# mbway/turbo

Hardware: AMD Instinct MI355X
Metric: acquisition evals/sec (M candidates, N training) + GP-fit ms (higher is better)
Workload: dtype f32

## Files before the change

turbo_amd/csrc/prune_screen_h2.hpp:

```cpp
#pragma once
#include <hip/hip_runtime.h>
#include <math.h>

#include "prune_screen.hpp"
#include "trmm_f16x2.hpp"

namespace tgp {

constexpr int SCRH_MIN_D = 15;
constexpr int SCRH_ROW = 144;
constexpr int SCRH_MAXEXP = 40;

struct ScreenH2Terms { double dcoef, P, Qc, Qw; };
inline ScreenH2Terms screen_h2_error_terms(double constant, int D, int N) {
    const double u = 0x1p-24, ce = 1.001 * constant, L = fabs(log2(constant));
    ScreenH2Terms t;
    t.dcoef = 2.01 * D + 25.0 + 0.26 * sqrt((double)D);
    t.P = ce * u * 0.5 * t.dcoef;
    t.Qc = screen_error_terms(constant, D, N).Q + ce * (0.7 * L * u + 0x1p-41);
    t.Qw = t.Qc + ce * u * (2.4 + 1.4 * L);
    return t;
}

__host__ __device__ inline double screen_h2_weight(double dcoef, double R) {
    const double delta = dcoef * 0x1p-24 * R + 0x1p-40;
    return delta <= 1.0 ? 1.001 * expm1(0.5001 * delta) : INFINITY;
}
__host__ __device__ inline double screen_h2_error(double closed, double wcoef, double W, double wadd) {
    return fmin(closed, wcoef * W + wadd);
}

__host__ __device__ inline float screen_h2_scale(float m) {
    int e;
    frexpf(m, &e);
    int ex = 14 - e;
    ex = ex > SCRH_MAXEXP ? SCRH_MAXEXP : (ex < -SCRH_MAXEXP ? -SCRH_MAXEXP : ex);
    return ldexpf(1.f, ex);
}

struct ScreenH2Scal {
    double ea, eb, wadd;
    float nxmax, sx;
    int npos, nneg, ok, pad;
};

struct ScreenH2PrepArgs {
    const float *Xs;
    const double *alpha;
    int N, Dp, nch;
    long ncap;
    double P, Qc, Qw;
    unsigned char *Xh;
    float *nxp, *absa;
    ScreenH2Scal *scal;
};

__global__ __launch_bounds__(256) void screen_h2_prep_kernel(ScreenH2PrepArgs a) {
    __shared__ double sa[256];
    __shared__ float smx[256], smn[256];
    __shared__ int spos[256], sbef[256], sbad[256];
    __shared__ int wcnt[4];
    const int tid = threadIdx.x, base = blockIdx.x * 256;
    const int N = a.N, Dp = a.Dp;
    double a1 = 0.0;
    float mxx = 0.f, mxn = 0.f;
    int npos = 0, before = 0, bad = 0;
    for (int i = tid; i < N; i += 256) {
        const float *row = a.Xs + (long)i * Dp;
        double s = 0.0;
        float m = 0.f;
        for (int d = 0; d < Dp; d += 4) {
            const f4_t x = *reinterpret_cast<const f4_t *>(row + d);
#pragma unroll
            for (int e = 0; e < 4; ++e) { s = fma((double)x[e], (double)x[e], s); m = fmaxf(m, fabsf(x[e])); }
        }
        if (!(s < (double)INFINITY)) bad = 1;
        mxn = fmaxf(mxn, (float)s);
        mxx = fmaxf(mxx, m);
        const double al = a.alpha[i];
        a1 += fabs(al);
        const int p = al >= 0.0;
        npos += p;
        if (i < base) before += p;
    }
    sa[tid] = a1; smx[tid] = mxx; smn[tid] = mxn; spos[tid] = npos; sbef[tid] = before; sbad[tid] = bad;
    __syncthreads();
    for (int o = 128; o > 0; o >>= 1) {
        if (tid < o) {
            sa[tid] += sa[tid + o];
            smx[tid] = fmaxf(smx[tid], smx[tid + o]);
            smn[tid] = fmaxf(smn[tid], smn[tid + o]);
            spos[tid] += spos[tid + o];
            sbef[tid] += sbef[tid + o];
            sbad[tid] |= sbad[tid + o];
        }
        __syncthreads();
    }
    npos = spos[0];
    before = sbef[0];
    const int nneg = N - npos, np128 = (npos + 127) & ~127, nn128 = (nneg + 127) & ~127;
    const float xm2 = 2.f * smx[0];
    const float sx = xm2 > 0.f ? screen_h2_scale(xm2) : 1.f;
    const int ok = !sbad[0] && xm2 < 0x1p54f;
    if (blockIdx.x == 0 && tid == 0) {
        const double an = 1.001 * sa[0];
        ScreenH2Scal s;
        s.ea = an * (a.P * (double)smn[0] + a.Qc);
        s.eb = an * a.P;
        s.wadd = an * a.Qw;
        s.nxmax = smn[0]; s.sx = sx;
        s.npos = npos; s.nneg = nneg; s.ok = ok; s.pad = 0;
        *a.scal = s;
    }

    const int i = base + tid;
    const bool live = i < N;
    const double al = live ? a.alpha[i] : -1.0;
    const bool pos = live && al >= 0.0;
    const unsigned long long bal = __ballot(pos);
    const int lane = tid & 63, w = tid >> 6;
    if (lane == 0) wcnt[w] = __popcll(bal);
    __syncthreads();
    int pre = __popcll(bal & ((1ull << lane) - 1ull));
    for (int k = 0; k < w; ++k) pre += wcnt[k];
    auto write_row = [&](long dest, const float *row, float absal) {
        double s = 0.0;
        for (int ch = 0; ch < a.nch; ++ch) {
            unsigned h[2][16];
#pragma unroll
            for (int q = 0; q < 8; ++q) {
                const int d = ch * SCR_DC + 4 * q;
                f4_t x = {0.f, 0.f, 0.f, 0.f};
                if (row && d < Dp) x = *reinterpret_cast<const f4_t *>(row + d);
#pragma unroll
                for (int e = 0; e < 4; ++e) s = fma((double)x[e], (double)x[e], s);
                split2_f16x2(-2.f * x[0], -2.f * x[1], sx, h[0][2 * q], h[1][2 * q]);
                split2_f16x2(-2.f * x[2], -2.f * x[3], sx, h[0][2 * q + 1], h[1][2 * q + 1]);
            }
            unsigned char *o = a.Xh + ((long)ch * a.ncap + dest) * 128;
#pragma unroll
            for (int pl = 0; pl < 2; ++pl)
#pragma unroll
                for (int q = 0; q < 4; ++q)
                    *reinterpret_cast<u4_t *>(o + 64 * pl + 16 * q) = (u4_t){h[pl][4 * q], h[pl][4 * q + 1], h[pl][4 * q + 2], h[pl][4 * q + 3]};
        }
        a.nxp[dest] = (float)s;
        a.absa[dest] = absal;
    };
    if (live) write_row(pos ? before + pre : np128 + (i - before - pre), a.Xs + (long)i * Dp, (float)fabs(al));
    if (blockIdx.x == 0 && tid < 128) {
        if (npos + tid < np128) write_row(npos + tid, nullptr, 0.f);
        if (nneg + tid < nn128) write_row(np128 + nneg + tid, nullptr, 0.f);
    }
}

struct ScreenH2Args {
    const float *Cs;
    const unsigned char *Xh;
    const float *nxp, *absa;
    const ScreenH2Scal *scal;
    double *mupart, *wpart;
    double *err, *wcoef;
    long ldpart, ncap;
    int Dp;
    double constant, dcoef;
};

__global__ __launch_bounds__(256, 2) void prune_screen_h2_kernel(ScreenH2Args g) {
    __shared__ __attribute__((aligned(16))) unsigned char Ct[SCR_T * SCRH_ROW];
    __shared__ __attribute__((aligned(16))) unsigned char Xt[SCR_T * SCRH_ROW];
    __shared__ __attribute__((aligned(16))) f4_t rowc[SCR_T];
    __shared__ float srow[SCR_T];
    __shared__ double mpos[SCR_T];
    const int tid = threadIdx.x, lane = tid & 63, w = tid >> 6;
    const int li = lane & 31, lh = lane >> 5;
    const long c0 = (long)blockIdx.x * SCR_T;
    const int Dp = g.Dp;
    const ScreenH2Scal sc = *g.scal;
    const int ntp = (sc.npos + SCR_T - 1) / SCR_T;
    const int njt = ntp + (sc.nneg + SCR_T - 1) / SCR_T;
    const int per = (njt + (int)gridDim.y - 1) / (int)gridDim.y;
    const int jt0 = blockIdx.y * per;
    const int jt1 = jt0 + per < njt ? jt0 + per : njt;
    const int nch = (Dp + SCR_DC - 1) / SCR_DC;
    const int nsteps = (jt1 > jt0 ? jt1 - jt0 : 0) * nch;
    const bool one_pass = nch == 1;
    constexpr float KAPPA = -0.72134752044448170368f;

    if (tid < SCR_T) {
        const float *row = g.Cs + (c0 + tid) * Dp;
        double s = 0.0;
        float m = 0.f;
        for (int d = 0; d < Dp; d += 4) {
            const f4_t x = *reinterpret_cast<const f4_t *>(row + d);
#pragma unroll
            for (int e = 0; e < 4; ++e) { s = fma((double)x[e], (double)x[e], s); m = fmaxf(m, fabsf(x[e])); }
        }
        const double R = s + (double)sc.nxmax;
        const bool ok = sc.ok && R < 0x1p46;
        const float sr = ok ? (m > 0.f ? screen_h2_scale(m) : 1.f) : 0.f;
        const float S = sr * sc.sx;
        srow[tid] = sr;
        rowc[tid] = (f4_t){S, KAPPA / S, (float)((double)log2f((float)g.constant) + (double)KAPPA * s), -(float)((double)S * s)};
        if (blockIdx.y == 0) {
            g.err[c0 + tid] = ok ? sc.ea + sc.eb * s : (double)INFINITY;
            g.wcoef[c0 + tid] = ok ? screen_h2_weight(g.dcoef, R) : (double)INFINITY;
        }
    }
    __syncthreads();
    ScrStage sp;
    u4_t xq[4];
    auto store_c = [&]() {
#pragma unroll
        for (int p = 0; p < 4; ++p) {
            const int idx = tid + 256 * p;
            const int r = idx >> 3, dv = (idx & 7) * 4;
            const float sr = srow[r];
            unsigned a0, a1, b0, b1;
            split2_f16x2(sp.v[p][0], sp.v[p][1], sr, a0, b0);
            split2_f16x2(sp.v[p][2], sp.v[p][3], sr, a1, b1);
            *reinterpret_cast<uint2 *>(Ct + r * SCRH_ROW + 2 * dv) = make_uint2(a0, a1);
            *reinterpret_cast<uint2 *>(Ct + r * SCRH_ROW + 64 + 2 * dv) = make_uint2(b0, b1);
        }
    };
    auto load_x = [&](int jt, int ch) {
        const unsigned char *src = g.Xh + ((long)ch * g.ncap + (long)jt * SCR_T) * 128;
#pragma unroll
        for (int p = 0; p < 4; ++p) xq[p] = *reinterpret_cast<const u4_t *>(src + (tid + 256 * p) * 16);
    };
    auto store_x = [&]() {
#pragma unroll
        for (int p = 0; p < 4; ++p) {
            const int idx = tid + 256 * p;
            *reinterpret_cast<u4_t *>(Xt + (idx >> 3) * SCRH_ROW + (idx & 7) * 16) = xq[p];
        }
    };
    if (nsteps > 0) {
        sp.load(g.Cs, c0, Dp, 0);
        load_x(jt0, 0);
        store_c();
        store_x();
    }
    __syncthreads();
    double sum[16];
#pragma unroll
    for (int r = 0; r < 16; ++r) sum[r] = 0.0;
    auto mma = [](u4_t a, u4_t b, f16_t c) {
        return __builtin_amdgcn_mfma_f32_32x32x16_f16(__builtin_bit_cast(f16x8_t, a), __builtin_bit_cast(f16x8_t, b), c, 0, 0, 0);
    };
    f16_t hi[4], mid[4];
    for (int st = 0; st < nsteps; ++st) {
        const int jt = jt0 + st / nch, ch = st - (st / nch) * nch;
        const int j0 = jt * SCR_T;
        const bool more = st + 1 < nsteps;
        if (more) {
            const int jn = jt0 + (st + 1) / nch, cn = (st + 1) - ((st + 1) / nch) * nch;
            load_x(jn, cn);
        }
        float nxv[4], al[4];
        if (ch == nch - 1) {
#pragma unroll
            for (int b = 0; b < 4; ++b) {
                nxv[b] = g.nxp[j0 + 32 * b + li];
                al[b] = g.absa[j0 + 32 * b + li];
            }
        }
        if (ch == 0) {
            if (jt == ntp && jt > jt0) {
#pragma unroll
                for (int r = 0; r < 16; ++r) {
                    double s = sum[r];
#pragma unroll
                    for (int o = 16; o > 0; o >>= 1) s += __shfl_xor(s, o, 64);
                    if (li == 0) mpos[32 * w + Mfma<float>::c_row(lane, r)] = s;
                    sum[r] = 0.0;
                }
            }
#pragma unroll
            for (int b = 0; b < 4; ++b)
#pragma unroll
                for (int r = 0; r < 16; ++r) { hi[b][r] = 0.f; mid[b][r] = 0.f; }
        }
        int dn = Dp - ch * SCR_DC;
        if (dn > SCR_DC) dn = SCR_DC;
        const int nkb = (dn + 15) >> 4;
#pragma unroll 1
        for (int kb = 0; kb < nkb; ++kb) {
            const int off = 32 * kb + 16 * lh;
            const unsigned char *ap = Ct + (32 * w + li) * SCRH_ROW + off;
            const u4_t a1 = *reinterpret_cast<const u4_t *>(ap), a2 = *reinterpret_cast<const u4_t *>(ap + 64);
#pragma unroll
            for (int b = 0; b < 4; ++b) {
                const unsigned char *bp = Xt + (32 * b + li) * SCRH_ROW + off;
                const u4_t b1 = *reinterpret_cast<const u4_t *>(bp), b2 = *reinterpret_cast<const u4_t *>(bp + 64);
                hi[b] = mma(a1, b1, hi[b]);
                mid[b] = mma(a1, b2, mid[b]);
                mid[b] = mma(a2, b1, mid[b]);
            }
        }
        if (ch == nch - 1) {
#pragma unroll
            for (int r = 0; r < 16; ++r) {
                const f4_t rc = rowc[32 * w + Mfma<float>::c_row(lane, r)];
                float p = 0.f;
#pragma unroll
                for (int b = 0; b < 4; ++b) {
                    const float t = fmaf(mid[b][r], 0x1p-11f, hi[b][r]);
                    const float s = fmaxf(fmaf(nxv[b], rc[0], t), rc[3]);
                    const float kv = __builtin_amdgcn_exp2f(fmaf(s, rc[1], rc[2]));
                    p = b == 0 ? kv * al[0] : fmaf(kv, al[b], p);
                }
                sum[r] += (double)p;
            }
        }
        if (more) {
            __syncthreads();
            if (!one_pass) {
                sp.load(g.Cs, c0, Dp, ((st + 1) - ((st + 1) / nch) * nch) * SCR_DC);
                store_c();
            }
            store_x();
            __syncthreads();
        }
    }
    const bool has_pos = nsteps > 0 && jt0 < ntp, has_neg = nsteps > 0 && jt1 > ntp;
#pragma unroll
    for (int r = 0; r < 16; ++r) {
        double s = sum[r];
#pragma unroll
        for (int o = 16; o > 0; o >>= 1) s += __shfl_xor(s, o, 64);
        if (li == 0) {
            const int row = 32 * w + Mfma<float>::c_row(lane, r);
            const double mp = has_neg ? (has_pos ? mpos[row] : 0.0) : s, mn = has_neg ? s : 0.0;
            const long o = (long)blockIdx.y * g.ldpart + c0 + row;
            g.mupart[o] = mp - mn;
            g.wpart[o] = mp + mn;
        }
    }
}

}
```

turbo_amd/csrc/sweep_pruned.hpp:

```cpp
#pragma once

namespace tgp {

struct BoundArgs {
    const double *mupart, *abspart; long ldpart; int njs;
    long m;
    double err_scale;
    const double *err;
    const double *wcoef;
    const double *wadd;
    double y_mean, y_std;
    double sig_lo, sig_hi;
    int acq; double sf, incumbent, param, margin;
    double *ub;
};

__global__ __launch_bounds__(256) void prune_bound_kernel(BoundArgs b) {
    const long c = (long)blockIdx.x * 256 + threadIdx.x;
    if (c >= b.m) return;
    double mun = 0.0, s = 0.0;
    for (int j = 0; j < b.njs; ++j) {
        mun += b.mupart[(long)j * b.ldpart + c];
        if (!b.err || b.wcoef) s += b.abspart[(long)j * b.ldpart + c];
    }
    double e = b.err ? b.err[c] : b.err_scale * s;
    if (b.wcoef) e = screen_h2_error(e, b.wcoef[c], s, b.wadd[0]);
    const double mu = b.y_std * (b.sf > 0.0 ? mun + e : mun - e) + b.y_mean;
    const double a_lo = acq_value(b.acq, b.sf, b.incumbent, b.param, mu, b.sig_lo);
    const double a_hi = acq_value(b.acq, b.sf, b.incumbent, b.param, mu, b.sig_hi);
    double a = a_lo > a_hi ? a_lo : a_hi;
    double scale = fabs(a);
    if (b.acq == TGP_ACQ_UCB) scale += fabs(mu) + fabs(b.param) * b.sig_hi;
    a += b.margin * scale;
    b.ub[c] = (isnan(a_lo) || isnan(a_hi) || isnan(a)) ? INFINITY : a;
}

__global__ __launch_bounds__(256) void prune_pick_kernel(const double *__restrict__ ub, long m, long gs,
                                                         long long *__restrict__ pick) {
    __shared__ double sv[256];
    __shared__ long long si[256];
    const long g0 = (long)blockIdx.x * gs;
    const long g1 = g0 + gs < m ? g0 + gs : m;
    Best b;
    for (long c = g0 + threadIdx.x; c < g1; c += 256) {
        const double u = ub[c];
        if (u > b.v) { b.v = u; b.i = c; }
    }
    b = block_argmax<256>(b, sv, si);
    if (threadIdx.x == 0) pick[blockIdx.x] = b.i == IDX_NONE ? g0 : b.i;
}

template <typename T>
__global__ __launch_bounds__(256) void prune_gather_kernel(const T *__restrict__ Cs, int Dp, const long long *__restrict__ idx,
                                                           long n, long rows, T *__restrict__ out) {
    const long total = rows * Dp;
    for (long i = (long)blockIdx.x * 256 + threadIdx.x; i < total; i += (long)gridDim.x * 256) {
        const long r = i / Dp;
        const int d = (int)(i - r * Dp);
        out[i] = r < n ? Cs[idx[r] * Dp + d] : (T)0;
    }
}

struct SurvArgs {
    const double *ub; long m;
    const long long *pick; long gs;
    const double *lb; double margin;
    int *bcnt; const int *boff;
    long long *sidx;
    const long long *src;
};

__device__ __forceinline__ bool prune_survives(const SurvArgs &s, long c) {
    const double lb = s.lb[0];
    const double bar = isinf(lb) ? lb : lb - s.margin * fabs(lb);
    return c < s.m && s.ub[c] >= bar && (s.src || s.pick[c / s.gs] != c);
}

__global__ __launch_bounds__(256) void prune_count_kernel(SurvArgs s) {
    __shared__ int wsum[4];
    const long c = (long)blockIdx.x * 256 + threadIdx.x;
    const unsigned long long bal = __ballot(prune_survives(s, c));
    if ((threadIdx.x & 63) == 0) wsum[threadIdx.x >> 6] = __popcll(bal);
    __syncthreads();
    if (threadIdx.x == 0) s.bcnt[blockIdx.x] = wsum[0] + wsum[1] + wsum[2] + wsum[3];
}

__global__ __launch_bounds__(1024) void prune_scan_kernel(const int *__restrict__ bcnt, int nb, int *__restrict__ boff,
                                                          long long *__restrict__ total) {
    __shared__ int part[1024];
    const int per = (nb + 1023) / 1024;
    const int b0 = (int)threadIdx.x * per;
    const int b1 = b0 + per < nb ? b0 + per : nb;
    int s = 0;
    for (int b = b0; b < b1; ++b) s += bcnt[b];
    part[threadIdx.x] = s;
    __syncthreads();
    for (int o = 1; o < 1024; o <<= 1) {
        const int v = (int)threadIdx.x >= o ? part[threadIdx.x - o] : 0;
        __syncthreads();
        part[threadIdx.x] += v;
        __syncthreads();
    }
    int run = part[threadIdx.x] - s;
    for (int b = b0; b < b1; ++b) { boff[b] = run; run += bcnt[b]; }
    if (threadIdx.x == 1023) total[0] = part[1023];
}

__global__ __launch_bounds__(256) void prune_scatter_kernel(SurvArgs s) {
    __shared__ int wsum[4];
    const long c = (long)blockIdx.x * 256 + threadIdx.x;
    const bool keep = prune_survives(s, c);
    const unsigned long long bal = __ballot(keep);
    const int lane = threadIdx.x & 63, w = threadIdx.x >> 6;
    if (lane == 0) wsum[w] = __popcll(bal);
    __syncthreads();
    int off = s.boff[blockIdx.x];
    for (int k = 0; k < w; ++k) off += wsum[k];
    if (keep) s.sidx[off + __popcll(bal & ((1ull << lane) - 1ull))] = s.src ? s.src[c] : c;
}

struct PruneWs {
    double *ub; long long *pick, *sidx, *misc; int *bcnt, *boff; void *cs;
    double *err, *ub1; long long *sidx1; float *nx;
    double *wcoef; unsigned char *xh; float *nxp, *absa; long ncap;
};
static size_t al256(size_t b) { return (b + 255) & ~(size_t)255; }

struct Carver {
    char *base = nullptr;
    size_t off = 0;
    template <typename U>
    U *take(size_t count, bool wanted = true) {
        U *ptr = base ? reinterpret_cast<U *>(base + off) : nullptr;
        if (wanted) off += al256(count * sizeof(U));
        return ptr;
    }
};

template <typename T>
static void prune_carve(const Context &c, int64_t npick, int64_t rows_cap, bool screen, bool h2, Carver &k, PruneWs &w) {
    const size_t M = (size_t)c.M, nb = (size_t)((c.M + 255) / 256), Mpad = (size_t)c.ws_Mpad;
    w.ncap = (long)((c.N + SCR_T - 1) / SCR_T + 1) * SCR_T;
    const size_t ncap = (size_t)w.ncap, nch = (size_t)((c.Dp + SCR_DC - 1) / SCR_DC);
    w.ub = k.take<double>(M);
    w.pick = k.take<long long>((size_t)npick);
    w.sidx = k.take<long long>(M);
    w.misc = k.take<long long>(32);
    w.bcnt = k.take<int>(nb);
    w.boff = k.take<int>(nb);
    w.cs = k.take<T>((size_t)rows_cap * c.Dp);
    w.err = k.take<double>(Mpad, screen);
    w.ub1 = k.take<double>((size_t)rows_cap, screen);
    w.sidx1 = k.take<long long>(M, screen);
    w.nx = k.take<float>((size_t)c.Np, screen);
    w.wcoef = k.take<double>(Mpad, h2);
    w.xh = k.take<unsigned char>(nch * ncap * 128, h2);
    w.nxp = k.take<float>(ncap, h2);
    w.absa = k.take<float>(ncap, h2);
}

template <typename T>
static hipError_t prune_workspace(Context &c, int64_t npick, int64_t rows_cap, bool screen, bool h2, PruneWs &w) {
    Carver count;
    prune_carve<T>(c, npick, rows_cap, screen, h2, count, w);
    TGP_TRY(c.d_prune.reserve(count.off, [&] { return hipStreamSynchronize(c.stream); }));
    Carver k{c.d_prune};
    prune_carve<T>(c, npick, rows_cap, screen, h2, k, w);
    return hipSuccess;
}

template <typename T>
static TrmmVariant contract_variant(const SweepPlan<T> &p, int64_t rows, int ntm) {
    TrmmVariant v;
    v.kern = p.early.kern; v.lds = trmm_glds_lds_bytes(); v.tile_m = 128; v.tile_n = 128; v.threads = 256;
    if ((rows / 128) * ntm >= CONTRACT_MIN_WGS) return v;
    if ((rows / 64) * ntm >= CONTRACT_MIN_WGS) {
        v.kern = trmm_sumsq_glds_narrow_kernel<T, 64>; v.lds = trmm_narrow_lds_bytes<64>(); v.tile_n = 64;
    } else {
        v.kern = trmm_sumsq_glds_narrow_kernel<T, 32>; v.lds = trmm_narrow_lds_bytes<32>(); v.tile_n = 32;
    }
    return v;
}

template <typename T>
static hipError_t contract_rows(Context &c, const SweepPlan<T> &p, const T *cs, int64_t n, ProfCursor &cur) {
    for (int64_t off = 0; off < n; off += c.launch_rows) {
        const int64_t m = n - off < c.launch_rows ? n - off : c.launch_rows;
        const int64_t rows = pad128(m);
        TGP_TRY(launch_kstar<T>(c, Kstar::SlabNoMean, cs + off * c.Dp, rows, p.njs, c.d_Ks[0].get(), c.d_mupart + off,
                                (long)c.Np / 16, 1.f, cur.st));
        cur.seg(1);
        TGP_TRY(launch_trmm<T>(c, p, contract_variant<T>(p, rows, p.n128), 0, off, rows, 0, p.n128, 0, true, cur.st));
        cur.seg(0, (double)m * (double)c.N * (double)c.N);
    }
    return hipSuccess;
}

enum class PruneGo { NotEligible, GatedOff, Go };
template <typename T>
static PruneGo prune_eligible(const Context &c, const SweepPlan<T> &p, const SweepCall &call) {
    const int acq = call.acq;
    if (call.mu || call.sigma || call.acqv) return PruneGo::NotEligible;
    if (acq != TGP_ACQ_EI && acq != TGP_ACQ_PI && acq != TGP_ACQ_UCB) return PruneGo::NotEligible;
    if (c.dtype != TGP_F32 && c.dtype != TGP_F64) return PruneGo::NotEligible;
    if (!p.mean_in_trmm || tuning_sweep_prune_now() == 0) return PruneGo::NotEligible;
    if (!(c.M > tuning().prune_top)) return PruneGo::NotEligible;
    if (!((double)c.M * (double)c.N * (double)c.N >= tuning_prune_min_work_now())) return PruneGo::NotEligible;
    const double u = sizeof(T) == 4 ? 0x1p-24 : 0x1p-53;
    const bool gate = c.noise > 0.0 && c.noise / (c.constant + c.noise) >= tuning().prune_tau * u;
    return gate ? PruneGo::Go : PruneGo::GatedOff;
}

template <typename T>
struct PruneRun {
    Context &c;
    const SweepPlan<T> &p;
    const SweepCall &call;
    PruneWs w;
    BoundArgs b;
    const T *Cs, *Xs;
    T *cs;
    int64_t gs, npick, keep;
    bool screen, h2;
    ProfCursor cur;
};

template <typename T>
static hipError_t tight_bound(PruneRun<T> &r, const T *rowsrc, int64_t rows, int64_t m, double *ub) {
    Context &c = r.c;
    const int njs_b = grid_splits(rows / (16 * kstar_ar(sizeof(T))), BOUND_MIN_WGS, r.p.njs, r.p.njs);
    TGP_TRY(launch_kstar<T>(c, Kstar::Bound, rowsrc, rows, njs_b, c.d_part.get(), c.d_mupart, 0L, 1.f, c.stream));
    r.cur.seg(1);
    r.b.njs = njs_b; r.b.m = m; r.b.err = nullptr; r.b.wcoef = nullptr; r.b.ub = ub;
    hipLaunchKernelGGL(prune_bound_kernel, dim3((unsigned)((m + 255) / 256)), dim3(256), 0, c.stream, r.b);
    return hipGetLastError();
}

static hipError_t screen_h2_bound(PruneRun<float> &r, int64_t xb, int njs_s) {
    Context &c = r.c;
    const PruneWs &w = r.w;
    const int N = (int)c.N, Dp = (int)c.Dp;
    const ScreenH2Terms et = screen_h2_error_terms(c.constant, (int)c.D, N);
    ScreenH2Scal *scal = reinterpret_cast<ScreenH2Scal *>(w.misc + 8);
    static_assert(sizeof(ScreenH2Scal) <= 256 - 64, "the scalars live behind misc's first eight words");
    ScreenH2PrepArgs a{};
    a.Xs = r.Xs; a.alpha = c.d_alpha; a.N = N; a.Dp = Dp; a.nch = (Dp + SCR_DC - 1) / SCR_DC; a.ncap = w.ncap;
    a.P = et.P; a.Qc = et.Qc; a.Qw = et.Qw;
    a.Xh = w.xh; a.nxp = w.nxp; a.absa = w.absa; a.scal = scal;
    hipLaunchKernelGGL(screen_h2_prep_kernel, dim3((unsigned)((N + 255) / 256)), dim3(256), 0, c.stream, a);
    TGP_TRY(hipGetLastError());
    r.cur.restart();
    ScreenH2Args g{};
    g.Cs = r.Cs; g.Xh = w.xh; g.nxp = w.nxp; g.absa = w.absa; g.scal = scal;
    g.mupart = c.d_mupart; g.wpart = c.d_part; g.err = w.err; g.wcoef = w.wcoef; g.ldpart = c.ws_Mpad; g.ncap = w.ncap;
    g.Dp = Dp; g.constant = c.constant; g.dcoef = et.dcoef;
    hipLaunchKernelGGL(prune_screen_h2_kernel, dim3((unsigned)xb, (unsigned)njs_s), dim3(256), 0, c.stream, g);
    TGP_TRY(hipGetLastError());
    r.cur.seg(2);
    c.prune_arith = 2;
    r.b.wcoef = w.wcoef; r.b.wadd = &scal->wadd;
    return hipSuccess;
}

static hipError_t screen_f32_bound(PruneRun<float> &r, int64_t xb, int njs_s) {
    Context &c = r.c;
    const PruneWs &w = r.w;
    const int N = (int)c.N, Dp = (int)c.Dp;
    const ScreenTerms et = screen_error_terms(c.constant, (int)c.D, N);
    double *scal = reinterpret_cast<double *>(w.misc + 8);
    hipLaunchKernelGGL(screen_stats_kernel, dim3(1), dim3(1024), 0, c.stream, r.Xs, c.d_alpha, N, (int)c.Np, Dp, et.P, et.Q, w.nx, scal);
    TGP_TRY(hipGetLastError());
    r.cur.restart();
    ScreenArgs g{};
    g.Cs = r.Cs; g.Xs = r.Xs; g.alpha = c.d_alpha; g.nx = w.nx; g.scal = scal;
    g.mupart = c.d_mupart; g.err = w.err; g.ldpart = c.ws_Mpad;
    g.N = N; g.Np = (int)c.Np; g.Dp = Dp; g.constant = c.constant;
    hipLaunchKernelGGL(prune_screen_kernel, dim3((unsigned)xb, (unsigned)njs_s), dim3(256), 0, c.stream, g);
    TGP_TRY(hipGetLastError());
    r.cur.seg(2);
    c.prune_arith = 1;
    r.b.wcoef = nullptr;
    return hipSuccess;
}

template <typename T>
static hipError_t bound_all(PruneRun<T> &r) {
    Context &c = r.c;
    if (!r.screen) return tight_bound<T>(r, r.Cs, c.ws_Mpad, c.M, r.w.ub);
    if constexpr (sizeof(T) == 4) {
        const int64_t xb = c.ws_Mpad / SCR_T;
        const int njt = ((int)c.N + SCR_T - 1) / SCR_T;
        const int njs_s = grid_splits(xb, SCREEN_MIN_WGS, r.p.njs, njt < r.p.njs ? njt : r.p.njs);
        TGP_TRY(r.h2 ? screen_h2_bound(r, xb, njs_s) : screen_f32_bound(r, xb, njs_s));
        r.b.njs = njs_s; r.b.m = c.M; r.b.err = r.w.err; r.b.ub = r.w.ub;
        hipLaunchKernelGGL(prune_bound_kernel, dim3((unsigned)((c.M + 255) / 256)), dim3(256), 0, c.stream, r.b);
        return hipGetLastError();
    }
    return hipSuccess;
}

template <typename T>
static hipError_t gather_rows(PruneRun<T> &r, const long long *idx, int64_t n) {
    const int Dp = (int)r.c.Dp;
    const long total = (long)pad128(n) * Dp;
    const long blocks = (total + 255) / 256 < 8192 ? (total + 255) / 256 : 8192;
    hipLaunchKernelGGL(prune_gather_kernel<T>, dim3((unsigned)blocks), dim3(256), 0, r.c.stream, r.Cs, Dp, idx, (long)n,
                       (long)pad128(n), r.cs);
    return hipGetLastError();
}

template <typename T>
static hipError_t finalize_rows(PruneRun<T> &r, const long long *idx, int64_t n, int64_t blk0) {
    FinArgs f = fin_args<T>(r.c, r.p, r.call);
    f.base_pairs = r.p.nunits;
    f.njs = 1;
    f.off = blk0 * FIN_BLOCK; f.m = n;
    f.gidx = idx;
    hipLaunchKernelGGL(finalize_kernel, dim3((unsigned)((n + FIN_BLOCK - 1) / FIN_BLOCK)), dim3(FIN_BLOCK), 0, r.c.stream, f);
    return hipGetLastError();
}

template <typename T>
static hipError_t lb_set(PruneRun<T> &r, int64_t &nblk) {
    Context &c = r.c;
    hipLaunchKernelGGL(prune_pick_kernel, dim3((unsigned)r.npick), dim3(256), 0, c.stream, r.w.ub, (long)c.M, (long)r.gs, r.w.pick);
    TGP_TRY(hipGetLastError());
    TGP_TRY(gather_rows(r, r.w.pick, r.npick));
    TGP_TRY(contract_rows<T>(c, r.p, r.cs, r.npick, r.cur));
    TGP_TRY(finalize_rows(r, r.w.pick, r.npick, 0));
    nblk = (r.npick + FIN_BLOCK - 1) / FIN_BLOCK;
    return launch_argmax(c, c.stream, (long)nblk, nullptr, nullptr, Bell{nullptr, 0, nullptr});
}

template <typename T>
static hipError_t survivors(PruneRun<T> &r, const double *ub, int64_t m, const long long *src, long long *out, long long &n) {
    Context &c = r.c;
    const PruneWs &w = r.w;
    hipStream_t st = c.stream;
    const int64_t nb = (m + 255) / 256;
    SurvArgs s{ub, (long)m, w.pick, (long)r.gs, c.d_best, r.b.margin, w.bcnt, w.boff, out, src};
    hipLaunchKernelGGL(prune_count_kernel, dim3((unsigned)nb), dim3(256), 0, st, s);
    TGP_TRY(hipGetLastError());
    hipLaunchKernelGGL(prune_scan_kernel, dim3(1), dim3(1024), 0, st, w.bcnt, (int)nb, w.boff, w.misc);
    TGP_TRY(hipGetLastError());
    hipLaunchKernelGGL(prune_scatter_kernel, dim3((unsigned)nb), dim3(256), 0, st, s);
    TGP_TRY(hipGetLastError());
    TGP_TRY(hipMemcpyAsync(&n, w.misc, sizeof(long long), hipMemcpyDeviceToHost, st));
    return hipStreamSynchronize(st);
}

template <typename T>
static hipError_t narrow_after_screen(PruneRun<T> &r, long long &nsurv, const long long *&sidx) {
    Context &c = r.c;
    const PruneWs &w = r.w;
    if (nsurv > r.keep) {
        r.cur.restart();
        TGP_TRY(tight_bound<T>(r, r.Cs, c.ws_Mpad, c.M, w.ub));
        TGP_TRY(survivors(r, w.ub, c.M, nullptr, w.sidx, nsurv));
    } else if (nsurv > tuning_prune_direct_now()) {
        TGP_TRY(gather_rows(r, w.sidx, nsurv));
        r.cur.restart();
        TGP_TRY(tight_bound<T>(r, r.cs, pad128(nsurv), nsurv, w.ub1));
        const long long n0 = nsurv;
        TGP_TRY(survivors(r, w.ub1, n0, w.sidx, w.sidx1, nsurv));
        sidx = w.sidx1;
    }
    r.cur.restart();
    return hipSuccess;
}

template <typename T>
static hipError_t contract_survivors_and_pick(PruneRun<T> &r, const long long *sidx, int64_t nsurv, int64_t nblk_lb) {
    int64_t nblk = 0;
    if (nsurv > 0) {
        TGP_TRY(gather_rows(r, sidx, nsurv));
        TGP_TRY(contract_rows<T>(r.c, r.p, r.cs, nsurv, r.cur));
        TGP_TRY(finalize_rows(r, sidx, nsurv, nblk_lb));
        nblk = (nsurv + FIN_BLOCK - 1) / FIN_BLOCK;
    }
    return launch_argmax(r.c, r.c.stream, (long)(nblk_lb + nblk), r.call.winner, r.call.res, Bell{nullptr, 0, nullptr});
}

static BoundArgs bound_args(const Context &c, const SweepCall &call, double margin) {
    BoundArgs b{};
    b.mupart = c.d_mupart; b.abspart = c.d_part; b.ldpart = c.ws_Mpad;
    b.err_scale = 4.0 * (double)((int)c.N + 8) * 0x1p-53;
    b.y_mean = c.y_mean; b.y_std = c.y_std;
    b.sig_lo = sqrt((0.99 * c.noise) * (c.y_std * c.y_std));
    b.sig_hi = sqrt((c.constant + c.noise) * (c.y_std * c.y_std));
    b.acq = call.acq; b.sf = call.sf; b.incumbent = call.incumbent; b.param = call.param; b.margin = margin;
    return b;
}

template <typename T>
static hipError_t sweep_pruned(Context &c, const SweepPlan<T> &p, const SweepCall &call, bool front_usable, bool &done) {
    done = false;
    const Tuning &tu = tuning();
    const int64_t M = c.M;
    const int64_t top = tu.prune_top < 1 ? 1 : tu.prune_top;
    const int64_t gs = (M + top - 1) / top, npick = (M + gs - 1) / gs;
    const double frac = tuning_prune_frac_now();
    const int64_t keep = frac < 0.0 ? -1 : (frac >= 1.0 ? M : (int64_t)(frac * (double)M));
    const int64_t rows_cap = pad128(npick > keep ? npick : keep);
    const bool screen = sizeof(T) == 4 && c.kernel == TGP_RBF && c.D <= SCR_MAXD && tuning_prune_screen_now() != 0;
    const bool h2 = screen && tuning_screen_arith_now() == 2 && c.D >= SCRH_MIN_D;
    PruneRun<T> r{c, p, call, PruneWs{}, BoundArgs{}, reinterpret_cast<const T *>(c.d_Cs.get()), train_points<T>(c), nullptr,
                  gs, npick, keep, screen, h2, ProfCursor{c, c.stream, -1}};
    TGP_TRY(prune_workspace<T>(c, npick, rows_cap, screen, h2, r.w));
    TGP_TRY(lds_opt_in(c, p.early.kern, p.early.lds));
    r.cs = reinterpret_cast<T *>(r.w.cs);
    c.prune_screen = -1;
    c.prune_arith = 0;
    if (!front_usable) TGP_TRY(issue_prep<T>(c, c.stream));
    r.cur.restart();
    r.b = bound_args(c, call, tu.prune_margin);

    TGP_TRY(bound_all(r));
    int64_t nblk_lb = 0;
    TGP_TRY(lb_set(r, nblk_lb));
    long long nsurv = 0;
    const long long *sidx = r.w.sidx;
    TGP_TRY(survivors(r, r.w.ub, M, nullptr, r.w.sidx, nsurv));
    c.prune_lbset = npick;
    if (screen) {
        c.prune_screen = nsurv;
        TGP_TRY(narrow_after_screen(r, nsurv, sidx));
    }
    c.prune_surv = nsurv;
    if (nsurv > keep) {
        c.prune_state = 1;
        return hipMemsetAsync(c.d_besti + 1, 0, sizeof(long long), c.stream);
    }
    TGP_TRY(contract_survivors_and_pick(r, sidx, nsurv, nblk_lb));
    c.prune_state = 0;
    done = true;
    return hipSuccess;
}

}
```

turbo_amd/csrc/tgp_internal.hpp:

```cpp
#pragma once
#include <hip/hip_runtime.h>
#include <stdint.h>

#include <string>
#include <vector>

#include "../../include/turbogp.h"
#include "dev_mem.hpp"
#include "doorbell.hpp"
#include "lds_opt_in.hpp"
#include "mes_math.hpp"
#include "tuning.hpp"

namespace tgp {


constexpr int NB = 64;
constexpr int NPAD = 256;
constexpr int SW_BM = 128;
constexpr int SW_BN = 128;
constexpr int KS_JS = 8;
constexpr int FIN_BLOCK = 256;
constexpr int CONTRACT_MIN_WGS = 512;
constexpr int SCREEN_MIN_WGS = 1024;
constexpr int BOUND_MIN_WGS = 2048;

struct ProfSeg { int a, b, kind; double flops; };

struct PreSweep {
    int mode = 0;
    int issue = 0;
    bool front = false;
    int rows128 = 0;
    long gen = -1;
    const double *cand = nullptr;
    int64_t M = 0, Mpad = 0, launch_rows = 0, chunk = 0;
    bool pending = false;
    Ev ev;
    Ev ev_in;
};

struct FitMem {
    Dev<double> d_t1, d_t2;
    Dev<double> d_Xs;
    Dev<double> d_ls;
    Dev<double> d_K;
    Dev<double> d_Linv;
    Dev<double> d_W;
    Dev<double> d_U;
    Dev<double> d_Dinv;
    Dev<double> d_Apan;
    Dev<double> d_yn;
    Dev<double> d_z;
    Dev<double> d_alpha;
    Dev<double> d_apart;
    Dev<float> d_Xs32;
    Dev<float> d_Linv32;
    Dev<unsigned short> d_Linv16;
    long linv16_gen = -1;
    Dev<unsigned> d_x2scal;
    int64_t cap_Np = 0, cap_D = 0;
    bool cap_full = false;
    int64_t linv_ld = 0;
    Dev<double> d_gpart;
    Dev<double> d_gout;
    int64_t g_cap_Np = 0, g_cap_Dp = 0;
    Dev<double> d_qws;
    Dev<double> d_rf;
    Dev<unsigned long long> d_stamp;
};

struct WsMem {
    Dev<void> d_Cs;
    Dev<void> d_Ks[2];
    Dev<double> d_part;
    Dev<double> d_mupart;
    int64_t ws_Mpad = 0;
    Dev<char> d_prune;
    Dev<double> d_topv;
    Dev<long long> d_topi;
    Dev<double> d_batch;
    Dev<double> d_bt;
    Dev<double> d_btm;
    Dev<long long> d_bti;
    Dev<double> d_ts;
    Dev<double> d_tsm;
    int64_t ts_S = 0, ts_F = 0;
    long ts_gen = -1;
    Dev<double> d_cov;
    Dev<double> d_mes;
    int mes_S = 0;
    long mes_gen = -1;
    Dev<double> d_int_a, d_int_mu, d_int_m2;
};

struct OutMem {
    Dev<double> d_mu, d_sigma, d_acq;
    int64_t out_cap = 0;
};

struct Context : FitMem, WsMem, OutMem {
    int device = 0;
    int dtype = TGP_F64;
    hipStream_t stream = nullptr;
    hipStream_t stream_own = nullptr;
    hipStream_t bg_lease = nullptr;
    hipStream_t stream_bg = nullptr;
    hipStream_t stream_pre = nullptr;
    PreSweep pre;
    std::vector<Ev> ev_la;
    Ev ev0, ev1;
    Ev evg[4];
    double last_grad_ms[3] = {0.0, 0.0, 0.0};
    std::string err;

    bool fitted = false;
    int64_t N = 0, D = 0, Np = 0;
    int64_t Dp = 0;
    int kernel = TGP_RBF;
    double constant = 1.0, noise = 0.0, jitter = 0.0;
    double y_mean = 0.0, y_std = 1.0, lml = 0.0;
    std::vector<double> ls;
    std::vector<double> h_X;
    std::vector<double> h_y;
    int normalize_y = 1;
    double sumlog = 0.0;
    Dev<double> d_scal;
    Dev<int> d_flag;
    bool grad_staged = false;
    bool grad_timed = true;
    double last_cov_ms = 0.0;
    long fit_gen = 0;
    float linv16_sb = 0.f;
    bool imported = false;
    int64_t import_rows = 0;
    int64_t fit_gen_src = -1;

    bool small = false;
    int64_t linv_extent = 0;
    Pin<double> h_pin_in{hipHostMallocMapped | hipHostMallocCoherent};
    Pin<double> h_pin_out{hipHostMallocMapped | hipHostMallocCoherent};
    Pin<double> h_pin_cand{hipHostMallocMapped};
    Pin<uint32_t> h_mt_words{hipHostMallocDefault, false};
    Ev ev_mt[2];
    Pin<unsigned long long> h_bell{hipHostMallocMapped | hipHostMallocCoherent};
    unsigned long long bell_seq = 0;
    Dev<unsigned> d_ticket;
    Dev<double> d_sfg;

    const double *d_cand = nullptr;
    Dev<double> d_cand_owned;
    int64_t M = 0;

    int64_t chunk = 0;
    int64_t launch_rows = 0;
    int prune_state = -1;
    int64_t prune_lbset = 0, prune_surv = 0;
    int64_t prune_screen = -1;
    int prune_arith = 0;
    double screen_ms = 0.0;
    Dev<double> d_bval;
    Dev<long long> d_bidx;
    double *d_winner = nullptr;
    int64_t winner_offset = 0;
    Ev ev_winner;
    bool winner_recorded = false;
    Dev<double> d_best;
    Dev<long long> d_besti;

    bool profiling = false;
    std::vector<Ev> ev_pool;
    size_t ev_used = 0;
    std::vector<ProfSeg> segs;
    int64_t trmm_launches = 0, kstar_launches = 0;
    double trmm_ms = 0.0, kstar_ms = 0.0;
    double trmm_flops = 0.0;
    double last_fit_ms = 0.0, last_sweep_ms = 0.0;
    int last_sweep_f64 = -1;
};

hipStream_t private_fit_begin(int device, bool may_borrow);
void private_fit_end(int device, bool held);
hipError_t launch_fit(Context &c, const double *staged_in, double *res_host, bool zero_linv = true, unsigned long long *start_stamp = nullptr);
hipError_t launch_ring(Context &c, const Bell &bell);
hipError_t device_streams(int device, hipStream_t *main, hipStream_t *bg, hipStream_t *pre = nullptr);
void device_streams_release(int device);
void device_stream_status(int device, int *bg_ok, int *pre_ok);
hipError_t launch_lml_grad(Context &c, bool ard, double *gout, bool timed = true);
hipError_t launch_f64_to_f32(Context &c, const double *in, float *out, long n);
constexpr int SMALL_GRAD_OUT_STRIDE = 72;
hipError_t launch_small_grad(Context &c, bool ard, double *out);
hipError_t launch_query(Context &c, const double *d_Xq, int m, int acq, double sf, double incumbent,
                        double param, double *d_ws, double *d_val, double *d_grad,
                        const Bell &bell = Bell{nullptr, 0, nullptr});
int64_t query_ws_doubles(const Context &c);
double *query_red(const Context &c, double *d_ws, int m);
hipError_t launch_gen_candidates(Context &c, double *dst, int64_t M, unsigned long long seed,
                                 unsigned long long first_candidate, const double *d_lo,
                                 const double *d_hi);
hipError_t launch_gen_lhs(Context &c, double *dst, int64_t M, int64_t D, unsigned long long seed,
                          unsigned long long first_sample, unsigned long long n_total,
                          const double *d_lo, const double *d_hi);
hipError_t launch_mt19937_columns(Context &c, const void *d_words, double *dst, int64_t M, const double *d_lo,
                                  const double *d_range);
hipError_t launch_fit_append(Context &c, int n_old);
hipError_t launch_topk(Context &c, const double *d_vals, long M, int k, double *ws_v, long long *ws_i,
                       long *final_off, double *done_host = nullptr, const Bell &bell = Bell{nullptr, 0, nullptr});
hipError_t launch_refine_clip(Context &c, double *d_xt, const double *d_lo, const double *d_hi, int R);
hipError_t launch_refine_step(Context &c, double *d_state, double *d_xt, const double *d_val,
                              const double *d_grad, const double *d_lo, const double *d_hi, int R,
                              int it, double pgtol, double ftol, int *d_active,
                              const double *d_red = nullptr, int acq = 0, double sf = 1.0, double incumbent = 0.0,
                              double param = 0.0);
hipError_t launch_refine_collect(Context &c, const double *d_state, int R, double *d_x, double *d_v, double *d_info);
long refine_state_stride(int D);
long refine_hist_doubles(int D, int R);
bool small_refine_fits(const Context &c);
hipError_t launch_small_refine(Context &c, const double *d_x0, const double *d_lo, const double *d_hi, int R,
                               int acq, double sf, double incumbent, double param, int max_iter,
                               double pgtol, double ftol, double *d_x, double *d_v, double *d_info);
hipError_t launch_small_query(Context &c, const double *d_xq, int m, int acq, double sf, double incumbent, double param,
                              double *d_val, double *d_grad, const Bell &bell);
hipError_t launch_small_fit(Context &c, const Bell &bell);
hipError_t launch_small_fit_grad(Context &c, bool ard, double *gout_host, const Bell &bell);
size_t small_fit_grad_ws_bytes();
long small_hyper_workspace_doubles(int N, int D, int Dp);
hipError_t launch_small_hyper(Context &c, int kernel, const double *d_X, const double *d_yn, const double *d_theta0,
                              const double *d_blo, const double *d_bhi, int S, int N, int D, int Dp, int n_ls,
                              int max_iter, double jitter, double *d_ws, double *d_theta, double *d_f, double *d_info,
                              bool one_wg_per_start = false);
size_t small_fit_args_bytes();
size_t small_sweep_args_bytes();
int64_t small_batch_ws_doubles(int64_t D, int64_t Dp);
int64_t mid_batch_ws_doubles(int64_t D, int64_t Dp);
void fill_mid_batch_args(void *fit_args, void *sweep_args, int64_t t, const double *in_dev, double *ws_dev,
                         double *res_dev, long long *counters_dev, const double *cand_dev, double *mu_dev,
                         double *sigma_dev, int64_t N, int64_t D, int64_t Dp, int64_t M, double constant,
                         double noise, double jitter, double y_mean, double y_std);
hipError_t launch_mid_batch(Context &c, int kernel, const void *fit_args_dev, const void *sweep_args_dev, int64_t T, int64_t M);
void fill_small_batch_args(void *fit_args, void *sweep_args, int64_t t, const double *in_dev, double *ws_dev,
                           double *res_dev, long long *counters_dev, const double *cand_dev, double *mu_dev,
                           double *sigma_dev, int64_t N, int64_t D, int64_t Dp, int64_t M, double constant,
                           double noise, double jitter, double y_mean, double y_std);
hipError_t launch_small_batch(Context &c, int kernel, const void *fit_args_dev, const void *sweep_args_dev,
                              int64_t T, int64_t M, bool fit, bool sweep);
struct SweepCall {
    int acq = TGP_ACQ_NONE;
    double sf = 1.0, incumbent = 0.0, param = 0.0;
    double *mu = nullptr, *sigma = nullptr, *acqv = nullptr;
    double *res = nullptr;
    double *winner = nullptr;
    Bell bell{nullptr, 0, nullptr};
    MesArgs mes{nullptr, 0, 0.0};
    bool may_use_front = false;
};
enum class SweepPath {
    OneWorkgroup,
    OneLaunch,
    General
};
int mid_sweep_cpw(const Context &c, int64_t M);
inline SweepPath sweep_path(const Context &c, int64_t M) {
    if (c.small && c.N <= 2 * NB) return SweepPath::OneWorkgroup;
    return mid_sweep_cpw(c, M) != 0 ? SweepPath::OneLaunch : SweepPath::General;
}
hipError_t launch_small_sweep(Context &c, const SweepCall &s);
hipError_t launch_argmax_final(Context &c, const SweepCall &s);
hipError_t launch_mid_sweep(Context &c, const SweepCall &s);
hipError_t launch_sweep(Context &c, const SweepCall &s, bool front_usable);
hipError_t presweep_front(Context &c, hipStream_t st);
hipError_t presweep_rows(Context &c, hipStream_t st, int rows_final, int budget128);

int prof_mark(Context &c, hipStream_t s);
void prof_seg(Context &c, int a, int b, int kind, double flops = 0.0);

constexpr int BT_MAXP = 64;
struct BtSmall {
    double *R;
    double *e;
    double *fant;
    double *inc;
    double *sel_val;
    long long *sel_idx;
    int *flag;
};
struct BatchWs {
    int64_t Mpad, nblk;
    int js;
    double *Zraw, *Zs, *Kz, *hw, *v, *w, *R, *selv;
    double *fant, *inc;
    double *e, *eps;
    double *Cs, *part, *bmu, *bvar, *bval, *G, *acqd;
    long long *seli, *clampw, *flagw, *bidx;
    unsigned char *mask;
};
hipError_t launch_query_front(Context &c, const double *d_xq, double *uq, double *ks, double *hw, double *v, double *w);
int bt_pass_splits(const Context &c, int64_t M);
hipError_t launch_bt_prep(Context &c, double *Cs, int64_t Mpad);
hipError_t launch_bt_init(Context &c, double *mu, double *var, unsigned char *mask);
hipError_t launch_bt_point(Context &c, const double *rec, const BtSmall &s, int k, double *zraw, unsigned char *mask);
struct McSmall;
hipError_t launch_bt_condition(Context &c, const BatchWs &ws, const BtSmall &s, const McSmall *mc, int j, int kb,
                               double lie, double sf);
hipError_t launch_bt_step(Context &c, const BatchWs &ws, const BtSmall &s, int j, int store, int acq, double sf,
                          double param, double *mu_out, double *sigma_out, int k);
constexpr int MC_MAXS = 64;
struct McSmall {
    BtSmall b;
    double *eps;
    double *fant;
    double *inc;
    int S;
};
hipError_t launch_mc_init(Context &c, const McSmall &s, int J, bool draw, unsigned long long seed, double incumbent);
hipError_t launch_mc_step(Context &c, const BatchWs &ws, const McSmall &s, int j, int acq, double sf, double param,
                          double *acq_out, double *sigma_out, int k);

struct TsDraw {
    int64_t S, F;
    double *omega;
    double *b;
    double *W;
    double *eps;
    double *V;
};
int ts_spad(int64_t S);
hipError_t launch_linv_solve(Context &c, const double *r, double *z, double *w, int m);
hipError_t launch_ts_draw(Context &c, const TsDraw &t, unsigned long long seed, double *priorX, double *R, double *Z);
hipError_t launch_ts_pass(Context &c, const TsDraw &t, const double *P, int64_t rows, bool update, double *out, double o0,
                          double o1);
hipError_t launch_ts_select(Context &c, const TsDraw &t, const double *f, double sf, int distinct, unsigned char *mask,
                            double *bval, long long *bidx, long long *sel_idx, double *sel_val, double *sel_x);
hipError_t launch_mes_take(Context &c, const double *src, int S, double sf, double incumbent, double *dst);
size_t ts_eval_lds_bytes(const Context &c, int64_t S);

struct CovWs {
    int64_t m, mpad, S, Spad, NV;
    int64_t o_cnt;
    int64_t o_Xq, o_Us, o_mu, o_dvec, o_Dinv, o_G;
    int64_t o_Ks, o_Vt;
    int64_t o_Ein, o_E, o_Y;
};
int64_t cov_ws_doubles(const Context &c, int64_t m, int64_t S, CovWs *out);
hipError_t launch_cov_posterior(Context &c, double *ws, const CovWs &w, int latent, double nugget, bool for_sample);
hipError_t launch_cov_sample(Context &c, double *ws, const CovWs &w, bool draw, unsigned long long seed);
hipError_t launch_ts_eval(Context &c, const TsDraw &t, const double *Xq, int m, double *fout, double *gout);

hipError_t launch_integrate_accumulate(Context &c, const SweepCall &s, int k);
hipError_t launch_integrate_final(Context &c, const SweepCall &s, int S);

}
```

Before: 81.92 million.

## Unroll screen prep rows, peel MFMA k-steps, and raise kstar splits in contraction

The prep kernel now processes four rows per thread per iteration so more independent loads are in flight. The screen kernel peels the k-loop into at most two explicit steps and starts the first chunk with a zero accumulator instead of a separate zeroing pass. It also makes the wave index uniform with readfirstlane. The contraction path now picks the kstar j-split count from a minimum workgroup target, so small row counts launch more workgroups. The peeled loop assumes nkb is at most 2, which holds only if SCR_DC is no larger than 32.

```diff
diff --git a/turbo_amd/csrc/prune_screen_h2.hpp b/turbo_amd/csrc/prune_screen_h2.hpp
--- a/turbo_amd/csrc/prune_screen_h2.hpp
+++ b/turbo_amd/csrc/prune_screen_h2.hpp
@@ -1,6 +1,8 @@
 #pragma once
 #include <hip/hip_runtime.h>
 #include <math.h>
+
+#include <type_traits>
 
 #include "prune_screen.hpp"
 #include "trmm_f16x2.hpp"
@@ -65,23 +67,38 @@
     double a1 = 0.0;
     float mxx = 0.f, mxn = 0.f;
     int npos = 0, before = 0, bad = 0;
-    for (int i = tid; i < N; i += 256) {
-        const float *row = a.Xs + (long)i * Dp;
-        double s = 0.0;
-        float m = 0.f;
+    for (int i0 = tid; i0 < N; i0 += 4 * 256) {
+        double s[4] = {0.0, 0.0, 0.0, 0.0}, al[4];
+        float m[4] = {0.f, 0.f, 0.f, 0.f};
+        const float *row[4];
+#pragma unroll
+        for (int q = 0; q < 4; ++q) {
+            const int i = i0 + 256 * q;
+            row[q] = a.Xs + (long)(i < N ? i : i0) * Dp;
+            al[q] = a.alpha[i < N ? i : i0];
+        }
         for (int d = 0; d < Dp; d += 4) {
-            const f4_t x = *reinterpret_cast<const f4_t *>(row + d);
-#pragma unroll
-            for (int e = 0; e < 4; ++e) { s = fma((double)x[e], (double)x[e], s); m = fmaxf(m, fabsf(x[e])); }
-        }
-        if (!(s < (double)INFINITY)) bad = 1;
-        mxn = fmaxf(mxn, (float)s);
-        mxx = fmaxf(mxx, m);
-        const double al = a.alpha[i];
-        a1 += fabs(al);
-        const int p = al >= 0.0;
-        npos += p;
-        if (i < base) before += p;
+            f4_t x[4];
+#pragma unroll
+            for (int q = 0; q < 4; ++q) x[q] = *reinterpret_cast<const f4_t *>(row[q] + d);
+#pragma unroll
+            for (int e = 0; e < 4; ++e)
+#pragma unroll
+                for (int q = 0; q < 4; ++q) { s[q] = fma((double)x[q][e], (double)x[q][e], s[q]); m[q] = fmaxf(m[q], fabsf(x[q][e])); }
+        }
+#pragma unroll
+        for (int q = 0; q < 4; ++q) {
+            const int i = i0 + 256 * q;
+            if (i < N) {
+                if (!(s[q] < (double)INFINITY)) bad = 1;
+                mxn = fmaxf(mxn, (float)s[q]);
+                mxx = fmaxf(mxx, m[q]);
+                a1 += fabs(al[q]);
+                const int p = al[q] >= 0.0;
+                npos += p;
+                if (i < base) before += p;
+            }
+        }
     }
     sa[tid] = a1; smx[tid] = mxx; smn[tid] = mxn; spos[tid] = npos; sbef[tid] = before; sbad[tid] = bad;
     __syncthreads();
@@ -172,7 +189,7 @@
     __shared__ __attribute__((aligned(16))) f4_t rowc[SCR_T];
     __shared__ float srow[SCR_T];
     __shared__ double mpos[SCR_T];
-    const int tid = threadIdx.x, lane = tid & 63, w = tid >> 6;
+    const int tid = threadIdx.x, lane = tid & 63, w = __builtin_amdgcn_readfirstlane(tid >> 6);
     const int li = lane & 31, lh = lane >> 5;
     const long c0 = (long)blockIdx.x * SCR_T;
     const int Dp = g.Dp;
@@ -249,6 +266,26 @@
         return __builtin_amdgcn_mfma_f32_32x32x16_f16(__builtin_bit_cast(f16x8_t, a), __builtin_bit_cast(f16x8_t, b), c, 0, 0, 0);
     };
     f16_t hi[4], mid[4];
+    auto kstep = [&](int kb, auto first_tag) {
+        constexpr bool FIRST = decltype(first_tag)::value;
+        const int off = 32 * kb + 16 * lh;
+        const unsigned char *ap = Ct + (32 * w + li) * SCRH_ROW + off;
+        const u4_t a1 = *reinterpret_cast<const u4_t *>(ap), a2 = *reinterpret_cast<const u4_t *>(ap + 64);
+#pragma unroll
+        for (int b = 0; b < 4; ++b) {
+            const unsigned char *bp = Xt + (32 * b + li) * SCRH_ROW + off;
+            const u4_t b1 = *reinterpret_cast<const u4_t *>(bp), b2 = *reinterpret_cast<const u4_t *>(bp + 64);
+            if constexpr (FIRST) {
+                const f16_t zero = {0.f, 0.f, 0.f, 0.f, 0.f, 0.f, 0.f, 0.f, 0.f, 0.f, 0.f, 0.f, 0.f, 0.f, 0.f, 0.f};
+                hi[b] = mma(a1, b1, zero);
+                mid[b] = mma(a1, b2, zero);
+            } else {
+                hi[b] = mma(a1, b1, hi[b]);
+                mid[b] = mma(a1, b2, mid[b]);
+            }
+            mid[b] = mma(a2, b1, mid[b]);
+        }
+    };
     for (int st = 0; st < nsteps; ++st) {
         const int jt = jt0 + st / nch, ch = st - (st / nch) * nch;
         const int j0 = jt * SCR_T;
@@ -265,39 +302,22 @@
                 al[b] = g.absa[j0 + 32 * b + li];
             }
         }
-        if (ch == 0) {
-            if (jt == ntp && jt > jt0) {
-#pragma unroll
-                for (int r = 0; r < 16; ++r) {
-                    double s = sum[r];
-#pragma unroll
-                    for (int o = 16; o > 0; o >>= 1) s += __shfl_xor(s, o, 64);
-                    if (li == 0) mpos[32 * w + Mfma<float>::c_row(lane, r)] = s;
-                    sum[r] = 0.0;
-                }
-            }
-#pragma unroll
-            for (int b = 0; b < 4; ++b)
-#pragma unroll
-                for (int r = 0; r < 16; ++r) { hi[b][r] = 0.f; mid[b][r] = 0.f; }
+        if (ch == 0 && jt == ntp && jt > jt0) {
+#pragma unroll
+            for (int r = 0; r < 16; ++r) {
+                double s = sum[r];
+#pragma unroll
+                for (int o = 16; o > 0; o >>= 1) s += __shfl_xor(s, o, 64);
+                if (li == 0) mpos[32 * w + Mfma<float>::c_row(lane, r)] = s;
+                sum[r] = 0.0;
+            }
         }
         int dn = Dp - ch * SCR_DC;
         if (dn > SCR_DC) dn = SCR_DC;
         const int nkb = (dn + 15) >> 4;
-#pragma unroll 1
-        for (int kb = 0; kb < nkb; ++kb) {
-            const int off = 32 * kb + 16 * lh;
-            const unsigned char *ap = Ct + (32 * w + li) * SCRH_ROW + off;
-            const u4_t a1 = *reinterpret_cast<const u4_t *>(ap), a2 = *reinterpret_cast<const u4_t *>(ap + 64);
-#pragma unroll
-            for (int b = 0; b < 4; ++b) {
-                const unsigned char *bp = Xt + (32 * b + li) * SCRH_ROW + off;
-                const u4_t b1 = *reinterpret_cast<const u4_t *>(bp), b2 = *reinterpret_cast<const u4_t *>(bp + 64);
-                hi[b] = mma(a1, b1, hi[b]);
-                mid[b] = mma(a1, b2, mid[b]);
-                mid[b] = mma(a2, b1, mid[b]);
-            }
-        }
+        if (ch == 0) kstep(0, std::true_type{});
+        else kstep(0, std::false_type{});
+        if (nkb == 2) kstep(1, std::false_type{});
         if (ch == nch - 1) {
 #pragma unroll
             for (int r = 0; r < 16; ++r) {
@@ -324,13 +344,14 @@
         }
     }
     const bool has_pos = nsteps > 0 && jt0 < ntp, has_neg = nsteps > 0 && jt1 > ntp;
+    const int elane = (int)__builtin_amdgcn_mbcnt_hi(~0u, __builtin_amdgcn_mbcnt_lo(~0u, 0u));
 #pragma unroll
     for (int r = 0; r < 16; ++r) {
         double s = sum[r];
 #pragma unroll
         for (int o = 16; o > 0; o >>= 1) s += __shfl_xor(s, o, 64);
-        if (li == 0) {
-            const int row = 32 * w + Mfma<float>::c_row(lane, r);
+        if ((elane & 31) == 0) {
+            const int row = 32 * w + Mfma<float>::c_row(elane, r);
             const double mp = has_neg ? (has_pos ? mpos[row] : 0.0) : s, mn = has_neg ? s : 0.0;
             const long o = (long)blockIdx.y * g.ldpart + c0 + row;
             g.mupart[o] = mp - mn;
diff --git a/turbo_amd/csrc/sweep_pruned.hpp b/turbo_amd/csrc/sweep_pruned.hpp
--- a/turbo_amd/csrc/sweep_pruned.hpp
+++ b/turbo_amd/csrc/sweep_pruned.hpp
@@ -187,7 +187,10 @@
     for (int64_t off = 0; off < n; off += c.launch_rows) {
         const int64_t m = n - off < c.launch_rows ? n - off : c.launch_rows;
         const int64_t rows = pad128(m);
-        TGP_TRY(launch_kstar<T>(c, Kstar::SlabNoMean, cs + off * c.Dp, rows, p.njs, c.d_Ks[0].get(), c.d_mupart + off,
+        const int ntile = (int)c.Np / 128;
+        const int njs_s = grid_splits(rows / (16 * kstar_ar(sizeof(T))), GATHER_KS_MIN_WGS, ntile, ntile);
+        const int njs_g = njs_s > p.njs ? njs_s : p.njs;
+        TGP_TRY(launch_kstar<T>(c, Kstar::SlabNoMean, cs + off * c.Dp, rows, njs_g, c.d_Ks[0].get(), c.d_mupart + off,
                                 (long)c.Np / 16, 1.f, cur.st));
         cur.seg(1);
         TGP_TRY(launch_trmm<T>(c, p, contract_variant<T>(p, rows, p.n128), 0, off, rows, 0, p.n128, 0, true, cur.st));
diff --git a/turbo_amd/csrc/tgp_internal.hpp b/turbo_amd/csrc/tgp_internal.hpp
--- a/turbo_amd/csrc/tgp_internal.hpp
+++ b/turbo_amd/csrc/tgp_internal.hpp
@@ -22,6 +22,7 @@
 constexpr int KS_JS = 8;
 constexpr int FIN_BLOCK = 256;
 constexpr int CONTRACT_MIN_WGS = 512;
+constexpr int GATHER_KS_MIN_WGS = 256;
 constexpr int SCREEN_MIN_WGS = 1024;
 constexpr int BOUND_MIN_WGS = 2048;
 
```

After: 84.59 million, median of 6. 3.3% higher.
